# sunjay/portrayer

Measured on AMD Instinct MI355X. Metric: Mray/s (primary+shadow+secondary) at 1920x1080 SAMPLES=64, higher is better.
Workload: dtype f64; 1 GPU; big-scene (1000 analytic primitives, 3 point lights, reference scene script) 1920x1080 SAMPLES=64; width=1920, height=1080, samples=64, traversal=flat, sampling=counter-based jitter, seed 0, partition=single GPU, rays_per_frame=367740795

## Files before the change

include/portrayer_hip.h:

```cpp
#ifndef PORTRAYER_HIP_H
#define PORTRAYER_HIP_H

#include <stdint.h>

#ifdef __cplusplus
extern "C" {
#endif

#define PT_ABI_VERSION 8

enum { PT_PRIM_SPHERE = 0, PT_PRIM_TRIANGLE = 1, PT_PRIM_MESH = 2, PT_PRIM_KDMESH = 3, PT_PRIM_PLANE = 4, PT_PRIM_CUBE = 5, PT_PRIM_CYLINDER = 6, PT_PRIM_CONE = 7 };
enum { PT_TRAVERSE_FLAT = 1, PT_TRAVERSE_KD = 2, PT_TRAVERSE_HIER = 3 };
enum { PT_SAMPLE_CENTRE = 0, PT_SAMPLE_RNG = 1 };

enum {
    PT_OK = 0,
    PT_ERR_ARGUMENT = -1,
    PT_ERR_DEVICE = -2,
    PT_ERR_NO_SCENE = -3,
    PT_ERR_SLICE = -4,
    PT_ERR_SCENE = -5,
    PT_ERR_TRAVERSAL = -6
};

// ... 363 lines not shown
int pt_copy_from_device(pt_context *ctx, void *dst, const void *src, uint64_t bytes);
int pt_synchronize(pt_context *ctx);
int pt_measure_copy_bandwidth(pt_context *ctx, uint64_t bytes, int iters, double *gbps);

int pt_test_cast_rays(pt_context *ctx, uint64_t n, const double *origins, const double *directions, int any_hit,
                      double *out_t, int32_t *out_node, int32_t *out_sub);
uint64_t pt_test_scene_bytes(const pt_context *ctx);
int pt_test_scene_info(const pt_context *ctx, uint64_t out[4]);
int pt_test_vertex_box_shape(const pt_context *ctx, uint64_t out[2]);
int pt_test_math(pt_context *ctx, int op, uint64_t n, const double *a, const double *b, double *out);
int pt_test_pow_host(uint64_t n, const double *x, const double *y, double *port, double *libm);
int pt_test_libm_host(int op, uint64_t n, const double *a, const double *b, double *out);
int pt_test_work_items(const pt_render_params *params, uint32_t *sample_count, uint64_t *sample_index_sum, uint32_t *chunk_length_sum,
                       uint64_t *n_items, uint32_t *lane_pixels_chunks_samples);
typedef struct pt_scene_traits {
    int32_t traverse;
    uint32_t n_nodes, n_lights;
    int32_t has_meshes;
    int32_t has_kdmesh;
    int32_t reflective;
    int32_t reflective_opaque;
    int32_t glossy;
    int32_t area_light;
    int32_t pad;
    uint64_t instanced_tris;
} pt_scene_traits;
int pt_test_kernel_choice(const pt_scene_traits *traits, int mode, int textured, uint32_t *kernel_mode, uint32_t *kernel_variant);
int pt_test_raypk(uint64_t n, int body, const double *origins, const double *directions, const double *t_max, const float *box_lo, const float *box_hi,
                  int32_t *verdict, float *t_near, float *t_far);
int pt_test_certain_shadow(uint64_t n, int type, const double *fwd, const double *inv, const double *P, const double *L, int32_t *out_certain, int32_t *out_exact_hit);
int pt_test_pixel_beam(uint64_t n, const double *cameras, const uint32_t *pixels, const double *jitters, const float *box_lo, const float *box_hi,
                       int32_t *accept, float *bound, int32_t *walk, double *rays);
int pt_test_pixel_list_summary(pt_context *ctx, uint64_t *out);
int pt_test_film_fold_host(uint32_t n, const double *samples, const uint32_t *cuts, uint32_t n_cuts, double out_sum[3]);
int pt_test_film_moments_host(uint32_t n, const double *samples, const uint32_t *cuts, uint32_t n_cuts, double out_sum[3], double *out_q, double *out_err);
int pt_test_film_plan_host(uint32_t width, uint32_t height, const pt_rect *slice, const uint32_t *budget, uint32_t max_samples, uint32_t round, uint32_t *list, uint32_t cap,
                           uint32_t *n_out);
int pt_test_film_plan(pt_context *ctx, uint32_t width, uint32_t height, const pt_rect *slice, const uint32_t *budget, uint32_t max_samples, uint32_t round, uint32_t *list, uint32_t cap,
                      uint32_t *n_out);
int pt_test_denoise_host(uint32_t width, uint32_t height, const pt_denoise_params *params, const double *linear, const double *variance, const uint32_t *counts,
                         const pt_denoise_guides *guides, double *out_linear, double *out_variance);
int pt_test_denoise_albedo_host(uint32_t width, uint32_t height, const pt_denoise_params *params, const double *linear, const double *variance, const uint32_t *counts,
                                const pt_denoise_guides *guides, const double *albedo, double *out_linear, double *out_variance);

#ifdef __cplusplus
}
#endif
#endif
```

portrayer_amd/_hip.py:

```python
from __future__ import annotations

import ctypes as C
import os
from typing import Optional

import numpy as np

PKG_DIR = os.path.dirname(os.path.abspath(__file__))
LIB_PATH = os.path.join(PKG_DIR, "libportrayer_hip.so")

TRAVERSE_FLAT, TRAVERSE_KD, TRAVERSE_HIER = 1, 2, 3
SAMPLE_CENTRE, SAMPLE_RNG = 0, 1
OK, ERR_ARGUMENT, ERR_DEVICE, ERR_NO_SCENE, ERR_SLICE, ERR_SCENE, ERR_TRAVERSAL = 0, -1, -2, -3, -4, -5, -6
KERNEL_WAVES_MASK, KERNEL_INTERPRETER, KERNEL_PARK, KERNEL_COUNTING, KERNEL_TEXTURED, KERNEL_FORK, KERNEL_CHAIN = 15, 16, 32, 64, 128, 256, 512

_dp = C.POINTER(C.c_double)
_ip = C.POINTER(C.c_int32)
_up = C.POINTER(C.c_uint32)
_u64p = C.POINTER(C.c_uint64)
_u8p = C.POINTER(C.c_uint8)


class PortrayerHipError(RuntimeError):
    pass
# ... 162 lines not shown
DENOISE_SAME_NODE = 1
DENOISE_ALBEDO_EPS = 0.0078125


class PtDenoiseParams(C.Structure):
    _fields_ = [("iterations", C.c_int32), ("flags", C.c_uint32), ("sigma_color", C.c_double), ("sigma_plane", C.c_double), ("normal_power_log2", C.c_int32)]


class PtDenoiseGuides(C.Structure):
    _fields_ = [("position", C.c_void_p), ("normal", C.c_void_p), ("node", C.c_void_p)]


class PtStats(C.Structure):
    _fields_ = [(n, C.c_uint64) for n in ("primary", "shadow", "reflect", "refract", "depth11_skipped", "hits", "n_inner", "n_leaf",
                                          "n_analytic", "n_tri", "n_bbox", "kd_plane_miss", "stack_overflow")] + \
               [("kernel_ms", C.c_double), ("total_ms", C.c_double), ("diag", C.c_uint64 * 8), ("kernel_mode", C.c_uint32), ("kernel_variant", C.c_uint32)]

    def as_dict(self):
        d = {n: (float if n.endswith("_ms") else int)(getattr(self, n)) for n, _ in self._fields_ if n != "diag"}
        d["diag"] = [int(x) for x in self.diag]
        return d


_lib: Optional[C.CDLL] = None

EXPORTS = ["pt_abi_version", "pt_device_count", "pt_context_create", "pt_context_destroy", "pt_last_error", "pt_scene_upload",
           "pt_render", "pt_render_device", "pt_render_finish", "pt_context_stream", "pt_context_next_slot", "pt_compact_bytes", "pt_untile_device", "pt_tile_slot_pixel", "pt_untile_host", "pt_device_alloc",
           "pt_device_free", "pt_copy_to_device", "pt_copy_from_device", "pt_synchronize", "pt_measure_copy_bandwidth", "pt_test_cast_rays",
           "pt_test_math", "pt_test_work_items", "pt_node_create", "pt_node_destroy", "pt_node_last_error", "pt_node_ranks", "pt_node_uses_rccl", "pt_node_context",
           "pt_node_scene_upload", "pt_node_render", "pt_node_upload_background", "pt_node_render_resident", "pt_node_download_image",
           "pt_node_device", "pt_node_frame_begin", "pt_node_frame_end", "pt_node_frames_in_flight", "pt_node_last_frame_host_ms", "pt_node_last_frame_rank_kernel_ms", "pt_test_pow_host", "pt_test_libm_host",
           "pt_aov", "pt_aov_device", "pt_aov_finish", "pt_rays", "pt_rays_device", "pt_rays_finish", "pt_segments", "pt_segments_device",
           "pt_radiance", "pt_radiance_device", "pt_radiance_finish", "pt_scene_update", "pt_node_scene_update", "pt_scene_deform", "pt_node_scene_deform", "pt_scene_mesh_rebuildable", "pt_test_scene_bytes", "pt_test_scene_info",
           "pt_vertex_bounds_device", "pt_scene_deform_device", "pt_test_vertex_box_shape", "pt_test_raypk", "pt_test_certain_shadow", "pt_test_pixel_beam", "pt_test_pixel_list_summary",
           "pt_film_create", "pt_film_destroy", "pt_film_reset", "pt_film_add", "pt_film_add_device", "pt_film_resolve", "pt_film_resolve_device", "pt_film_counts",
           "pt_test_film_fold_host",
           "pt_film_create_moments", "pt_film_add_map", "pt_film_add_map_device", "pt_film_error", "pt_film_error_device", "pt_film_budget_device",
           "pt_test_film_moments_host", "pt_test_film_plan_host", "pt_test_film_plan",
           "pt_film_denoise", "pt_film_denoise_device", "pt_test_denoise_host",
           "pt_guides", "pt_guides_device", "pt_guides_finish", "pt_film_denoise_albedo", "pt_film_denoise_albedo_device", "pt_test_denoise_albedo_host",
           "pt_ao", "pt_ao_device", "pt_ao_finish", "pt_test_ao_rays_host", "pt_test_ao_tables",
           "pt_gather", "pt_gather_device", "pt_gather_finish", "pt_test_kernel_choice",
           "pt_chart_triangles", "pt_chart", "pt_chart_device", "pt_test_chart_host",
           "pt_direct", "pt_direct_device", "pt_direct_finish", "pt_test_direct_host"]


def header_functions():
    import re
    with open(os.path.join(os.path.dirname(os.path.dirname(os.path.abspath(__file__))), "include", "portrayer_hip.h")) as fh:
        text = re.sub(r"/\*.*?\*/", "", fh.read(), flags=re.S)
    return sorted(set(re.findall(r"\b(pt_[a-z0-9_]+)\s*\(", text)))


def missing_symbols():
    l = lib()
    return [n for n in header_functions() if not hasattr(l, n)]


def lib() -> C.CDLL:
    global _lib
    if _lib is None:
        if not os.path.exists(LIB_PATH):
            raise PortrayerHipError(f"{LIB_PATH} is missing: build it with `make` (or __graft_entry__.build()); there is no CPU fallback")
        l = C.CDLL(LIB_PATH)
        l.pt_abi_version.restype = C.c_int
        l.pt_device_count.restype = C.c_int
        l.pt_context_create.restype = C.c_int
# ... 36 lines not shown
        l.pt_context_next_slot.argtypes = [C.c_void_p]
        l.pt_compact_bytes.restype = C.c_uint64
        l.pt_compact_bytes.argtypes = [C.POINTER(PtRenderParams)]
        l.pt_untile_device.restype = C.c_int
        l.pt_untile_device.argtypes = [C.c_void_p, C.POINTER(PtRenderParams), C.c_void_p, C.c_void_p, C.c_void_p]
        l.pt_tile_slot_pixel.restype = C.c_int
        l.pt_tile_slot_pixel.argtypes = [C.POINTER(PtRenderParams), C.c_uint32, C.c_uint32, _up, _up]
        l.pt_untile_host.restype = C.c_int
        l.pt_untile_host.argtypes = [C.POINTER(PtRenderParams), _u8p, _u8p]
        l.pt_device_alloc.restype = C.c_int
        l.pt_device_alloc.argtypes = [C.c_void_p, C.c_uint64, C.POINTER(C.c_void_p)]
        l.pt_device_free.restype = C.c_int
        l.pt_device_free.argtypes = [C.c_void_p, C.c_void_p]
        l.pt_copy_to_device.restype = C.c_int
        l.pt_copy_to_device.argtypes = [C.c_void_p, C.c_void_p, C.c_void_p, C.c_uint64]
        l.pt_copy_from_device.restype = C.c_int
        l.pt_copy_from_device.argtypes = [C.c_void_p, C.c_void_p, C.c_void_p, C.c_uint64]
        l.pt_synchronize.restype = C.c_int
        l.pt_synchronize.argtypes = [C.c_void_p]
        l.pt_measure_copy_bandwidth.restype = C.c_int
        l.pt_measure_copy_bandwidth.argtypes = [C.c_void_p, C.c_uint64, C.c_int, _dp]
        l.pt_test_cast_rays.restype = C.c_int
        l.pt_test_cast_rays.argtypes = [C.c_void_p, C.c_uint64, _dp, _dp, C.c_int, _dp, _ip, _ip]
        l.pt_test_work_items.restype = C.c_int
        l.pt_test_work_items.argtypes = [C.c_void_p, C.POINTER(C.c_uint32), C.POINTER(C.c_uint64), C.POINTER(C.c_uint32), C.POINTER(C.c_uint64), C.POINTER(C.c_uint32)]
        l.pt_test_certain_shadow.restype = C.c_int
        l.pt_test_certain_shadow.argtypes = [C.c_uint64, C.c_int, _dp, _dp, _dp, _dp, _ip, _ip]
        l.pt_test_raypk.restype = C.c_int
        l.pt_test_raypk.argtypes = [C.c_uint64, C.c_int, _dp, _dp, _dp, C.POINTER(C.c_float), C.POINTER(C.c_float), _ip, C.POINTER(C.c_float), C.POINTER(C.c_float)]
        l.pt_test_pixel_list_summary.restype = C.c_int
        l.pt_test_pixel_list_summary.argtypes = [C.c_void_p, C.POINTER(C.c_uint64)]
        l.pt_test_pixel_beam.restype = C.c_int
        l.pt_test_pixel_beam.argtypes = [C.c_uint64, _dp, C.POINTER(C.c_uint32), _dp, C.POINTER(C.c_float), C.POINTER(C.c_float), _ip, C.POINTER(C.c_float), _ip, _dp]
        l.pt_test_math.restype = C.c_int
        l.pt_test_math.argtypes = [C.c_void_p, C.c_int, C.c_uint64, _dp, _dp, _dp]
        l.pt_node_create.restype = C.c_int
        l.pt_node_create.argtypes = [C.c_int, _ip, C.POINTER(C.c_void_p)]
        l.pt_node_destroy.restype = None
        l.pt_node_destroy.argtypes = [C.c_void_p]
        l.pt_node_last_error.restype = C.c_char_p
        l.pt_node_last_error.argtypes = [C.c_void_p]
        l.pt_node_ranks.restype = C.c_int
        l.pt_node_ranks.argtypes = [C.c_void_p]
        l.pt_node_uses_rccl.restype = C.c_int
        l.pt_node_uses_rccl.argtypes = [C.c_void_p]
        l.pt_node_context.restype = C.c_void_p
        l.pt_node_context.argtypes = [C.c_void_p, C.c_int]
        l.pt_node_scene_upload.restype = C.c_int
        l.pt_node_scene_upload.argtypes = [C.c_void_p, C.POINTER(PtScene), C.c_int, C.POINTER(PtKdTree)]
        l.pt_node_render.restype = C.c_int
        l.pt_node_render.argtypes = [C.c_void_p, C.POINTER(PtCamera), _dp, C.POINTER(PtRenderParams), _u8p, C.POINTER(PtStats)]
        l.pt_node_upload_background.restype = C.c_int
        l.pt_node_upload_background.argtypes = [C.c_void_p, _dp, C.POINTER(PtRenderParams), _u8p]
        l.pt_node_render_resident.restype = C.c_int
        l.pt_node_render_resident.argtypes = [C.c_void_p, C.POINTER(PtCamera), C.POINTER(PtRenderParams), C.POINTER(PtStats)]
        l.pt_node_download_image.restype = C.c_int
        l.pt_node_download_image.argtypes = [C.c_void_p, C.POINTER(PtRenderParams), _u8p]
        l.pt_node_device.restype = C.c_int
        l.pt_node_device.argtypes = [C.c_void_p, C.c_int]
        l.pt_node_frame_begin.restype = C.c_int
        l.pt_node_frame_begin.argtypes = [C.c_void_p, C.POINTER(PtCamera), C.POINTER(PtRenderParams)]
        l.pt_node_frame_end.restype = C.c_int
        l.pt_node_frame_end.argtypes = [C.c_void_p, C.POINTER(PtStats)]
        l.pt_node_frames_in_flight.restype = C.c_int
        l.pt_node_frames_in_flight.argtypes = [C.c_void_p]
        l.pt_node_last_frame_host_ms.restype = C.c_int
# ... 195 lines not shown
```

portrayer_amd/csrc/pt_api.hip:

```cpp
#include <type_traits>

#include "pt_context.h"
#include "pt_aov_inst.h"
#include "pt_guides_inst.h"
#include "pt_chart.h"
#include "pt_rays_inst.h"
#include "pt_segments_inst.h"
#include "pt_ao_inst.h"
#include "pt_direct_inst.h"
#include "pt_radiance_inst.h"
#include "pt_gather_inst.h"
#include "pt_film_inst.h"
#include "pt_film_map_inst.h"
#include "pt_denoise.h"
#include "pt_render_inst.h"
#include "pt_shade.h"
#include "pt_pixel_list.h"

template <int MODE>
__global__ void __launch_bounds__(PT_BLOCK) pt_cast_kernel(PtSceneView sc, uint64_t n, const double* o, const double* d, int any,
                                                          double* out_t, int32_t* out_node, int32_t* out_sub, unsigned int* overflow) {
    extern __shared__ uint32_t pt_lds[];
    PtStack stk;
    stk.base = pt_lds + threadIdx.x;
// ... 78 lines not shown
    PtRenderArgs r = a;
    r.tile_rank = i / slots_per_rank;
    uint32_t w = i % slots_per_rank, x, y;
    if (!pt_slot_to_pixel(r, w, &x, &y)) return;
    const uint8_t* s = gathered + 3 * (size_t)i;
    uint8_t* d = rgb + 3 * ((size_t)y * a.width + x);
    d[0] = s[0]; d[1] = s[1]; d[2] = s[2];
}

__global__ void __launch_bounds__(256) pt_occ_seed_kernel(uint32_t* __restrict__ occ, uint32_t n, int hashed, uint64_t seed, uint32_t all, uint32_t n_nodes) {
    const uint32_t i = blockIdx.x * blockDim.x + threadIdx.x;
    if (i >= n) return;
    occ[i] = hashed ? (uint32_t)(pt_rng_key(seed, i) % ((uint64_t)n_nodes + 1u)) : all + 1u;
}

__global__ void __launch_bounds__(256) pt_eye_table_kernel(const double* __restrict__ inv, double* __restrict__ tab, uint32_t n_nodes, double ex, double ey, double ez) {
    const uint32_t i = blockIdx.x * blockDim.x + threadIdx.x;
    if (i >= n_nodes) return;
    const double* m = inv + 12 * (size_t)i;
    double* o = tab + 12 * (size_t)i;
    const PtVec3 e = pt_xform_point(m, pt_v3(ex, ey, ez));
    o[0] = m[0]; o[1] = m[1]; o[2] = m[2]; o[3] = e.x;
    o[4] = m[4]; o[5] = m[5]; o[6] = m[6]; o[7] = e.y;
    o[8] = m[8]; o[9] = m[9]; o[10] = m[10]; o[11] = e.z;
}

__global__ void __launch_bounds__(256) pt_certain_table_kernel(const uint32_t* __restrict__ info, const double* __restrict__ fwd, const double* __restrict__ inv, float* __restrict__ tab,
                                                               uint32_t n_nodes) {
    const uint32_t i = blockIdx.x * blockDim.x + threadIdx.x;
    if (i >= n_nodes) return;
    pt_certain_ball(info[4 * (size_t)i], fwd + 12 * (size_t)i, inv + 12 * (size_t)i, tab + 4 * (size_t)i);
}

#define PT_PL_BLOCK 256
#define PT_PL_STACK 64
__global__ void __launch_bounds__(PT_PL_BLOCK) pt_pixel_list_kernel(PtRenderArgs a, uint32_t* __restrict__ table, uint32_t cap) {
    __shared__ uint32_t s_list[PT_PL_BLOCK / 64][PT_PL_K][64];
    __shared__ uint32_t s_stack[PT_PL_BLOCK / 64][PT_PL_STACK];
    const uint32_t wave = threadIdx.x >> 6, lane = threadIdx.x & 63u;
    const uint32_t tile_local = blockIdx.x * (PT_PL_BLOCK / 64) + wave;
    if (tile_local >= a.n_slots / 64u) return;
    const PtSceneView& sc = a.scene;
    const uint32_t slot = tile_local * 64u + lane;
    uint32_t x, y;
    pt_slot_to_pixel(a, slot, &x, &y);
    const PtBeam beam = pt_beam_setup(a.cam, (double)x, (double)y);
    uint32_t* const list = &s_list[wave][0][lane];
    uint32_t* const stack = s_stack[wave];
    uint32_t count = 0, tail = PT_PL_INF_BITS;
    if (cap > PT_PL_K) cap = PT_PL_K;
    bool overflowed = false;
    int sp = 0;
    auto add_leaf = [&](uint32_t ref, bool reached, float bound) {
        const uint32_t first = (ref & ~PT_REF_LEAF) >> 3, n = (ref & 7u) + 1u;
        for (uint32_t i = 0; i < n; i++) {
            const uint32_t node = sc.tlas_direct ? first : sc.bvh_items[first + i];
            if (reached) pt_pl_insert(list, 64u, cap, &count, &tail, pt_pl_entry(bound, node));
        }
    };
    const uint32_t root = sc.tlas_root;
    if (sc.n_nodes != 0 && root != PT_REF_EMPTY) {
        if (root & PT_REF_LEAF) add_leaf(root, true, 0.0f);
        else { stack[0] = root; sp = 1; }
    }
    while (sp > 0) {
        __builtin_amdgcn_fence(__ATOMIC_RELEASE, "wavefront");
        __builtin_amdgcn_wave_barrier();
        __builtin_amdgcn_fence(__ATOMIC_ACQUIRE, "wavefront");
        const uint32_t cur = (uint32_t)__builtin_amdgcn_readfirstlane((int)stack[sp - 1]);
        sp--;
        const pt_u32x16 nd = pt_sload_node(sc.bvh, cur);
#pragma unroll
        for (int ch = 0; ch < 2; ch++) {
            const uint32_t ref = nd[12 + ch];
            if (ref == PT_REF_EMPTY) continue;
            float lo[3], hi[3], bound = 0.0f;
#pragma unroll
            for (int k = 0; k < 3; k++) { lo[k] = pt_f32_of(nd[2 * k + ch]); hi[k] = pt_f32_of(nd[6 + 2 * k + ch]); }
            const bool reached = pt_beam_box(beam, lo, hi, &bound);
            if (!__any(reached)) continue;
            if (ref & PT_REF_LEAF) add_leaf(ref, reached, bound);
            else if (sp < PT_PL_STACK) { if (lane == 0) stack[sp] = ref; sp++; }
            else overflowed = true;
        }
    }
    uint32_t* rec = table + (size_t)slot * PT_PL_WORDS;
    uint32_t wds[PT_PL_WORDS];
    wds[0] = overflowed ? PT_PL_WALK : count;
    wds[1] = tail;
#pragma unroll
    for (uint32_t k = 0; k < PT_PL_K; k++) wds[2 + k] = k < count ? list[k * 64u] : 0u;
#pragma unroll
    for (uint32_t k = 0; k < PT_PL_WORDS; k += 4) reinterpret_cast<uint4*>(rec)[k / 4] = make_uint4(wds[k], wds[k + 1], wds[k + 2], wds[k + 3]);
}

#define PT_PASS_MISC_BYTES (256 + PT_FINE_QUEUES * PT_QUEUE_STRIDE * 4)
static size_t pt_stack_column(const PtSceneView& sc, int stack_lds_cap);

static int pt_pass_prepare(pt_context* c, PtPass& v) {
    if (v.ev0) return PT_OK;
    PT_HIP(c, hipEventCreate(&v.ev0));
    PT_HIP(c, hipEventCreate(&v.ev1));
    PT_HIP(c, hipEventCreateWithFlags(&v.copy_done, hipEventDisableTiming));
    PT_HIP(c, hipHostMalloc((void**)&v.host, 256, hipHostMallocDefault));
    return PT_OK;
}

static int pt_pass_open(pt_context* c, PtPass& v, PtRenderArgs& r, uint32_t grid, bool frames, hipStream_t stream) {
    r.n_lanes = grid * PT_BLOCK;
    int rc;
    if ((rc = pt_reserve(c, v.stack_spill, (size_t)r.n_lanes * pt_stack_column(r.scene, r.stack_lds_cap) * 4))) return rc;
    if (frames && (rc = pt_reserve(c, v.spill, pt_needs_spill(c->traits) ? (size_t)r.n_lanes * PT_SPILL_DEPTHS * PT_SPILL_STRIDE * sizeof(double) : 16))) return rc;
    if ((rc = pt_reserve(c, v.misc, PT_PASS_MISC_BYTES))) return rc;
    r.stack_spill = (uint32_t*)v.stack_spill.p;
    if (frames) r.spill = (double*)v.spill.p;
    r.overflow_flag = (unsigned int*)v.misc.p + 1;
    r.work_queues = (unsigned int*)((char*)v.misc.p + 256);
    r.fine_queues = 16;
    v.stream = stream; v.queued = true; v.closed = false;
    PT_HIP(c, hipMemsetAsync(v.misc.p, 0, PT_PASS_MISC_BYTES, stream));
    PT_HIP(c, hipEventRecord(v.ev0, stream));
    return PT_OK;
}

static int pt_pass_seal(pt_context* c, PtPass& v) {
    PT_HIP(c, hipEventRecord(v.ev1, v.stream));
    PT_HIP(c, hipMemcpyAsync(v.host, v.misc.p, 8, hipMemcpyDeviceToHost, v.stream));
// ... 259 lines not shown
            }
        }
        if (m0) v |= 2;
        if (o0) v |= 4;
        if ((m0 != 0) != (m1 != 0) || (o0 != 0) != (o1 != 0)) v |= 8;
        verdict[i] = v;
    }
    return PT_OK;
}

extern "C" int pt_test_pixel_list_summary(pt_context* c, uint64_t* out) {
    if (!c || !out) return PT_ERR_ARGUMENT;
    for (uint32_t k = 0; k < 5u + PT_PL_K; k++) out[k] = 0;
    if (c->pl_slot < 0 || c->pl_slots == 0) return PT_OK;
    PT_HIP(c, hipSetDevice(c->device));
    PT_HIP(c, hipDeviceSynchronize());
    std::vector<uint32_t> rec((size_t)c->pl_slots * PT_PL_WORDS);
    const pt_context::Slot& sl = c->slot[c->pl_slot];
    if (sl.eye_tab.bytes < c->pl_off + rec.size() * 4) return pt_fail(c, PT_ERR_ARGUMENT, "the slot's buffer no longer holds that launch's lists");
    PT_HIP(c, hipMemcpy(rec.data(), (const char*)sl.eye_tab.p + c->pl_off, rec.size() * 4, hipMemcpyDeviceToHost));
    out[0] = c->pl_slots;
    for (uint32_t i = 0; i < c->pl_slots; i++) {
        const uint32_t head = rec[(size_t)i * PT_PL_WORDS], tail = rec[(size_t)i * PT_PL_WORDS + 1];
        if (head & PT_PL_WALK) { out[3]++; continue; }
        const uint32_t n = head & 255u;
        if (n > PT_PL_K) return pt_fail(c, PT_ERR_TRAVERSAL, "a pixel list longer than its record");
        if (n == 0 && tail == PT_PL_INF_BITS) out[1]++;
        if (tail != PT_PL_INF_BITS) out[2]++;
        out[4 + n]++;
    }
    return PT_OK;
}

extern "C" int pt_test_pixel_beam(uint64_t n, const double* cameras, const uint32_t* pixels, const double* jitters, const float* box_lo, const float* box_hi,
                                  int32_t* accept, float* bound, int32_t* walk, double* rays) {
    if (!cameras || !pixels || !jitters || !box_lo || !box_hi || !accept || !bound || !walk) return PT_ERR_ARGUMENT;
    for (uint64_t i = 0; i < n; i++) {
        PtCamera cam;
        const double* cp = cameras + 19 * i;
        for (int k = 0; k < 3; k++) cam.eye[k] = cp[k];
        for (int k = 0; k < 12; k++) cam.view_to_world[k] = cp[3 + k];
        cam.fov_factor = cp[15]; cam.aspect = cp[16]; cam.width = cp[17]; cam.height = cp[18];
        const uint32_t x = pixels[2 * i], y = pixels[2 * i + 1];
        const float* lo = box_lo + 3 * i;
        const float* hi = box_hi + 3 * i;
        const PtBeam beam = pt_beam_setup(cam, (double)x, (double)y);
        float b = 0.0f;
        accept[i] = pt_beam_box(beam, lo, hi, &b) ? 1 : 0;
        bound[i] = accept[i] ? b : 0.0f;
        const PtRay r = pt_camera_ray(cam, (double)x + jitters[2 * i], (double)y + jitters[2 * i + 1]);
        if (rays) { rays[6 * i] = r.o.x; rays[6 * i + 1] = r.o.y; rays[6 * i + 2] = r.o.z; rays[6 * i + 3] = r.d.x; rays[6 * i + 4] = r.d.y; rays[6 * i + 5] = r.d.z; }
        PtRayPk q;
        int s[3];
        s[0] = pt_raypk_axis(r.o.x, r.d.x, &q.a[0], &q.b[0]); s[1] = pt_raypk_axis(r.o.y, r.d.y, &q.a[1], &q.b[1]); s[2] = pt_raypk_axis(r.o.z, r.d.z, &q.a[2], &q.b[2]);
        pt_u32x16 rec;
        for (int k = 0; k < 16; k++) rec[k] = 0u;
        for (int k = 0; k < 3; k++) {
            uint32_t l, h;
            memcpy(&l, lo + k, 4); memcpy(&h, hi + k, 4);
            rec[2 * k] = rec[2 * k + 1] = l; rec[6 + 2 * k] = rec[6 + 2 * k + 1] = h;
        }
        unsigned long long m0 = 0, m1 = 0, first = 0, o0 = 0, o1 = 0;
        pt_slab_pk2<PT_OCT_MIXED>(rec, q, INFINITY, &m0, &m1, &first);
        o0 = m0; o1 = m1;
        if (s[0] && s[1] && s[2]) {
            switch ((s[0] == 2 ? 1 : 0) | (s[1] == 2 ? 2 : 0) | (s[2] == 2 ? 4 : 0)) {
                case 0: pt_slab_pk2<0>(rec, q, INFINITY, &o0, &o1, &first); break;
                case 1: pt_slab_pk2<1>(rec, q, INFINITY, &o0, &o1, &first); break;
                case 2: pt_slab_pk2<2>(rec, q, INFINITY, &o0, &o1, &first); break;
                case 3: pt_slab_pk2<3>(rec, q, INFINITY, &o0, &o1, &first); break;
                case 4: pt_slab_pk2<4>(rec, q, INFINITY, &o0, &o1, &first); break;
                case 5: pt_slab_pk2<5>(rec, q, INFINITY, &o0, &o1, &first); break;
                case 6: pt_slab_pk2<6>(rec, q, INFINITY, &o0, &o1, &first); break;
                default: pt_slab_pk2<7>(rec, q, INFINITY, &o0, &o1, &first); break;
            }
        }
        walk[i] = (m0 ? 1 : 0) | (o0 ? 2 : 0);
    }
    return PT_OK;
}

extern "C" int pt_test_certain_shadow(uint64_t n, int type, const double* fwd, const double* inv, const double* P, const double* L, int32_t* out_certain, int32_t* out_exact_hit) {
    if (!fwd || !inv || !P || !L || !out_certain || !out_exact_hit || type < 0 || type > 7) return PT_ERR_ARGUMENT;
    for (uint64_t i = 0; i < n; i++) {
        float ball[4];
        pt_certain_ball((uint32_t)type, fwd + 12 * i, inv + 12 * i, ball);
        const PtVec3 p = pt_v3(P[3 * i], P[3 * i + 1], P[3 * i + 2]), l = pt_v3(L[3 * i], L[3 * i + 1], L[3 * i + 2]);
        out_certain[i] = ball[3] > 0.0f && pt_certain_lane(ball, (float)p.x, (float)p.y, (float)p.z, (float)l.x, (float)l.y, (float)l.z) ? 1 : 0;
        PtRay r;
        r.o = p;
        const PtVec3 hit_to_light = l - p;
        r.d = hit_to_light / pt_length(hit_to_light);
        const PtRay local = pt_ray_to_local(inv + 12 * i, r);
        double t;
        uint32_t part = 0;
        out_exact_hit[i] = pt_unit_prim_hit((uint32_t)type, local, PT_EPSILON, INFINITY, &t, &part) ? 1 : 0;
    }
    return PT_OK;
}

static bool pt_kd_semantics(int mode) { return mode == PT_MODE_KD || mode == PT_MODE_KD_NOMESH || mode == PT_MODE_KD_MESH; }
static int pt_stack_lds_cap(const PtSceneView& sc, size_t block_budget, size_t frame_bytes) {
    int lds_cap = block_budget > frame_bytes ? (int)((block_budget - frame_bytes) / (PT_BLOCK * 4)) : 0;
    lds_cap = std::max(lds_cap, 2);
    if (const char* e = getenv("PORTRAYER_LDS_STACK")) lds_cap = std::max(1, atoi(e));
    int cap = std::min(lds_cap, sc.stack_cap);
    if (pt_kd_semantics(sc.mode)) cap = std::max(cap, (sc.stack_cap + 63) / 64 + 2);
    return cap;
}
static size_t pt_stack_column(const PtSceneView& sc, int stack_lds_cap) {
    const int wave_rows = std::min(std::max(8, (sc.stack_cap + 63) / 64), std::max(stack_lds_cap, 8));
// ... 152 lines not shown
        }
        occ_seed = true;
    }
    if ((rc = pt_reserve(c, sl.misc, misc_head + occ_bytes))) return rc;
    if ((rc = pt_reserve(c, sl.accum, (size_t)a.n_slots * a.n_chunks * 3 * sizeof(double)))) return rc;
    a.accum = (double*)sl.accum.p;
#ifndef PT_NO_EYE_TABLE
    const bool eye_table = a.scene.mode == PT_MODE_FLAT_NOMESH && a.scene.n_nodes > 0;
#else
    const bool eye_table = false;
#endif
#ifndef PT_NO_CERTAIN_SHADOW
    const bool certain_table = a.scene.mode == PT_MODE_FLAT_NOMESH && a.scene.n_nodes > 0 && occ_bytes != 0;
#else
    const bool certain_table = false;
#endif
#ifndef PT_NO_PIXEL_LISTS
    const bool list_header = eye_table;
#ifdef PT_PIXEL_LIST_STATS
    const bool list_reader = true;
#else
    const bool list_reader = !stats;
#endif
    bool pixel_lists = eye_table && list_reader && (a.run_variant == PT_RUN_LINE3 || a.run_variant == PT_RUN_LINE4 || a.run_variant == PT_RUN_LINE5) && a.k_log2 + a.c_log2 == 6u &&
                       a.scene.n_nodes <= PT_PL_MAX_NODES && a.n_slots != 0;
    if (const char* e = getenv("PORTRAYER_PIXEL_LISTS")) if (atoi(e) <= 0) pixel_lists = false;
    uint32_t list_cap = PT_PL_K;
    if (const char* e = getenv("PORTRAYER_PIXEL_LIST_CAP"); e && *e) {
        char* end = nullptr;
        const unsigned long long k = strtoull(e, &end, 10);
        if (end == e || *end || k > PT_PL_K) return pt_fail(c, PT_ERR_ARGUMENT, std::string("PORTRAYER_PIXEL_LIST_CAP=") + e + ": expected 0 .. " + std::to_string(PT_PL_K));
        list_cap = (uint32_t)k;
    }
#else
    const bool list_header = false, pixel_lists = false;
    const uint32_t list_cap = 0;
#endif
    const size_t list_off = pt_pl_header_offset((uint32_t)a.scene.n_nodes);
    a.eye_tab = nullptr;
    if (eye_table || certain_table) {
        if ((rc = pt_reserve(c, sl.eye_tab, list_header ? list_off + pt_pl_bytes(pixel_lists ? a.n_slots : 0u) : (size_t)a.scene.n_nodes * (12 * sizeof(double) + 4 * sizeof(float))))) return rc;
        a.eye_tab = (const double*)sl.eye_tab.p;
    }
    a.spill = (double*)sl.spill.p;
    a.stack_spill = (uint32_t*)sl.stack_spill.p;
    a.work_counter = (unsigned int*)sl.misc.p;
    a.overflow_flag = (unsigned int*)sl.misc.p + 1;
    a.counters = (PtCounters*)((char*)sl.misc.p + 256);
    a.work_queues = (unsigned int*)((char*)sl.misc.p + 256 + sizeof(PtCounters));
    a.occluders = occ_bytes ? (uint32_t*)((char*)sl.misc.p + misc_head) : nullptr;
    a.occ_row = std::max<uint32_t>(a.div_tiles_x.d / std::max<uint32_t>(a.tile_ranks, 1u), 1u);
    c->last_mode = (uint32_t)a.scene.mode;
    c->last_variant = pt_choice_variant(choice, tex) | (stats ? PT_KERNEL_COUNTING : 0u);
    PT_HIP(c, hipMemsetAsync(sl.misc.p, 0, misc_head + occ_bytes, stream));
    if (occ_seed) {
        const uint32_t n_occ = (uint32_t)(occ_bytes / 4);
        hipLaunchKernelGGL(pt_occ_seed_kernel, dim3((n_occ + 255) / 256), dim3(256), 0, stream, a.occluders, n_occ, occ_hashed ? 1 : 0, occ_seed_value, occ_all, a.scene.n_nodes);
        PT_HIP(c, hipGetLastError());
        if (getenv("PORTRAYER_VERBOSE")) fprintf(stderr, "[pt_render] occluder table: %u entries seeded (PORTRAYER_OCC_SEED=%s)\n", n_occ, getenv("PORTRAYER_OCC_SEED"));
    }
    sl.mode = c->last_mode; sl.variant = c->last_variant; sl.counted = stats;
    PT_HIP(c, hipEventRecord(sl.ev0, stream));
    if (a.n_items) {
        if (eye_table) {
            hipLaunchKernelGGL(pt_eye_table_kernel, dim3((a.scene.n_nodes + 255) / 256), dim3(256), 0, stream, a.scene.inv, (double*)sl.eye_tab.p, (uint32_t)a.scene.n_nodes,
                               a.cam.eye[0], a.cam.eye[1], a.cam.eye[2]);
            PT_HIP(c, hipGetLastError());
        }
        if (certain_table) {
            hipLaunchKernelGGL(pt_certain_table_kernel, dim3((a.scene.n_nodes + 255) / 256), dim3(256), 0, stream, a.scene.info, a.scene.fwd, a.scene.inv, (float*)((double*)sl.eye_tab.p + 12 * (size_t)a.scene.n_nodes),
                               (uint32_t)a.scene.n_nodes);
            PT_HIP(c, hipGetLastError());
        }
        if (list_header) {
            uint32_t* const header = (uint32_t*)((char*)sl.eye_tab.p + list_off);
            PT_HIP(c, hipMemsetD32Async((hipDeviceptr_t)header, pixel_lists ? 1 : 0, 16, stream));
            if (pixel_lists) {
                const uint32_t tiles = a.n_slots / 64u;
                hipLaunchKernelGGL(pt_pixel_list_kernel, dim3((tiles + PT_PL_BLOCK / 64 - 1) / (PT_PL_BLOCK / 64)), dim3(PT_PL_BLOCK), 0, stream, a, header + 16, list_cap);
                PT_HIP(c, hipGetLastError());
            }
        }
        c->pl_slot = pixel_lists ? slot_index : -1; c->pl_slots = a.n_slots; c->pl_off = list_off + 64;
        PT_HIP(c, pt_dispatch(a, stats, c->n_cu, stream, &grid, true));
        hipLaunchKernelGGL(pt_finish_kernel, dim3((a.n_slots + PT_BLOCK - 1) / PT_BLOCK), dim3(PT_BLOCK), 0, stream, a);
        PT_HIP(c, hipGetLastError());
    }
    PT_HIP(c, hipEventRecord(sl.ev1, stream));
    PT_HIP(c, hipMemcpyAsync(sl.host, sl.misc.p, stats ? PT_SLOT_BYTES : 8, hipMemcpyDeviceToHost, stream));
    PT_HIP(c, hipEventRecord(sl.copy_done, stream));
    return PT_OK;
}

static int pt_collect_stats(pt_context* c, pt_stats* st, int slot_index) {
    pt_context::Slot& sl = c->slot[slot_index];
    if (st) memset(st, 0, sizeof *st);
    unsigned int head[2];
    memcpy(head, sl.host, sizeof head);
    if (st) {
        float ms = 0.f;
        PT_HIP(c, hipEventElapsedTime(&ms, sl.ev0, sl.ev1));
        st->kernel_ms = ms;
        if (sl.counted) {
            PtCounters h;
            memcpy(&h, sl.host + 256, sizeof h);
            st->primary = h.primary; st->shadow = h.shadow; st->reflect = h.reflect; st->refract = h.refract;
            st->depth11_skipped = h.depth11_skipped; st->hits = h.hits; st->n_inner = h.n_inner; st->n_leaf = h.n_leaf;
            st->n_analytic = h.n_analytic; st->n_tri = h.n_tri; st->n_bbox = h.n_bbox; st->kd_plane_miss = h.kd_plane_miss;
            st->stack_overflow = h.stack_overflow;
            for (int k = 0; k < 8; k++) st->diag[k] = h.diag[k];
        }
        if (head[1] && !st->stack_overflow) st->stack_overflow = 1;
        st->kernel_mode = sl.mode; st->kernel_variant = sl.variant;
    }
    if (head[1] & 2u) return pt_fail(c, PT_ERR_TRAVERSAL, "fork / join of refracted subtrees stalled (a lane waited for a colour nobody was computing): results invalid");
    if (head[1] & 4u) return pt_fail(c, PT_ERR_TRAVERSAL, "a tree walk did not end (watchdog): results invalid");
// ... 1581 lines not shown
```

portrayer_amd/csrc/pt_context.h:

```cpp
#pragma once
#include <hip/hip_runtime.h>

#include <algorithm>
#include <chrono>
#include <cmath>
#include <cstdio>
#include <cstring>
#include <string>
#include <vector>

#include "../../include/portrayer_hip.h"
#include "pt_build.h"
#include "pt_bvh.h"
#include "pt_shade.h"

struct PtBuf {
    void* p = nullptr;
    size_t bytes = 0;
    PtBuf() = default;
    PtBuf(const PtBuf&) = delete;
    PtBuf& operator=(const PtBuf&) = delete;
    ~PtBuf() { if (p) hipFree(p); }
};

// ... 27 lines not shown
struct pt_film;
struct pt_context {
    int device = 0;
    int n_cu = 0;
    std::string err;
    PtBuf inv, fwd, nrm, info, tri_v, tri_e, tri_leaf, tri_n, meshes, materials, lights, bvh, bvh4, bvh_items, kd, kd_items;
    PtBuf mat_maps, uv_trans, tex, tex_rgb, srgb_lut, tri_uv, texview, mkd, mkd_items;
    PtBuf node_box, kd_box, mkd_box, mkd_item_box, kd_ref;
    PtBuf g_inv, g_fwd, g_nrm, chain_off, chain, dfs_rank, hier_rec, own_inv;
    PtBuf bg, rgb, linear, misc;
    PtSceneTraits traits = {};
    uint32_t launch_seq = 0;
    PtSceneView view;
    bool have_scene = false;
    struct Slot {
        PtBuf spill, stack_spill, accum, misc;
        PtBuf eye_tab;
        hipStream_t stream = nullptr;
        hipEvent_t ev0 = nullptr, ev1 = nullptr;
        hipEvent_t copy_done = nullptr;
        unsigned char* host = nullptr;
        bool pending = false, counted = false;
        uint32_t mode = 0, variant = 0;
        std::chrono::steady_clock::time_point t_start;
    };
    static constexpr int PT_SLOTS = 2;
    Slot slot[PT_SLOTS];
    int slot_next = 0;
    int slot_oldest = 0;
    uint32_t last_mode = 0, last_variant = 0;
    int pl_slot = -1;
    uint32_t pl_slots = 0;
    size_t pl_off = 0;
    struct Aov {
        PtPass pass;
        PtBuf out[6];
        PtBuf albedo;
        bool guides = false;
        PtBuf chart_owner, chart_uv, chart_covered;
        bool chart = false;
    } aov;
    struct Rays {
        PtPass pass;
        PtBuf in[2], in_t_max, out[7];
        PtRaySort sort;
    } rays;
    struct Radiance {
        PtPass pass;
        PtBuf in[3], out;
        PtRaySort sort;
    } radiance;
    PtPass* const passes[3] = {&aov.pass, &rays.pass, &radiance.pass};
    std::vector<pt_film*> films;
    pt_film* film_open = nullptr;
    struct Resident {
        int traverse = 0;
        uint32_t n_nodes = 0, n_graph = 0, n_lights = 0;
        std::vector<uint32_t> info;
        std::vector<PtBuildBox> mesh_box;
        std::vector<PtBuildBox> tri_box;
        size_t mesh_tris = 0;
        std::vector<uint32_t> chain_off, chain;
        size_t tlas_first = 0, tlas_cap = 0;
        size_t tlas_items = 0;
        size_t tree_nodes = 0;
        int tlas_leaf = 1, collapse_mode = 1;
// ... 62 lines not shown
```

portrayer_amd/csrc/pt_pixel_list.h:

```cpp
#pragma once

#include "pt_scene_view.h"

#ifndef PT_PL_K
#define PT_PL_K 6u
#endif
#define PT_PL_WORDS (PT_PL_K <= 6u ? 8u : 16u)
static_assert(PT_PL_K >= 1u && PT_PL_K <= 14u, "a record is 8 or 16 words: head, tail bound, entries");
#define PT_PL_WALK 0x80000000u
#define PT_PL_MAX_NODES 65536u
#define PT_PL_INF_BITS 0x7F800000u

PT_HD size_t pt_pl_header_offset(uint32_t n_nodes) { return ((size_t)n_nodes * (12 * sizeof(double) + 4 * sizeof(float)) + 63u) & ~(size_t)63u; }
PT_HD size_t pt_pl_bytes(uint32_t n_slots) { return 64u + (size_t)n_slots * (PT_PL_WORDS * 4u); }

struct PtBeamAxis {
    int neg;
    float a1, a2;
    float be1, be2;
    float bf1, bf2;
};
struct PtBeam {
    PtBeamAxis ax[3];
    float lmin;
};

PT_HD float pt_f32_below(double v) {
    float f = (float)v;
    if ((double)f > v) {
        const uint32_t u = __builtin_bit_cast(uint32_t, f);
        f = f > 0.0f ? __builtin_bit_cast(float, u - 1u) : (f < 0.0f ? __builtin_bit_cast(float, u + 1u) : -1.401298464324817e-45f);
    }
    return f;
}
PT_HD float pt_f32_above(double v) { return -pt_f32_below(-v); }

PT_HD double pt_beam_view_x(const PtCamera& c, double x) {
    double ndc_x = x / c.width;
    return (2.0 * ndc_x - 1.0) * c.aspect * c.fov_factor;
}
PT_HD double pt_beam_view_y(const PtCamera& c, double y) {
    double ndc_y = y / c.height;
    return (1.0 - 2.0 * ndc_y) * c.fov_factor;
}
PT_HD void pt_beam_corner(const PtCamera& c, double view_x, double view_y, double D[3]) {
    PtVec3 eye = pt_v3(c.eye[0], c.eye[1], c.eye[2]);
    PtVec3 world = pt_xform_point(c.view_to_world, pt_v3(view_x, view_y, -1.0));
    PtVec3 d = world - eye;
    D[0] = d.x; D[1] = d.y; D[2] = d.z;
}

PT_HD PtBeam pt_beam_setup(const PtCamera& c, double px, double py) {
    double lo[3], hi[3];
    bool finite = true;
    const double vx[2] = {pt_beam_view_x(c, px), pt_beam_view_x(c, px + 1.0)}, vy[2] = {pt_beam_view_y(c, py), pt_beam_view_y(c, py + 1.0)};
    for (int k = 0; k < 4; k++) {
        double D[3];
        pt_beam_corner(c, vx[k & 1], vy[k >> 1], D);
        for (int a = 0; a < 3; a++) {
            finite = finite && fabs(D[a]) < INFINITY;
            if (k == 0) { lo[a] = hi[a] = D[a]; }
            else { lo[a] = fmin(lo[a], D[a]); hi[a] = fmax(hi[a], D[a]); }
        }
    }
    double lmax2 = 0.0, lmin2 = 0.0;
    for (int a = 0; a < 3; a++) {
        const double m = fmax(fabs(lo[a]), fabs(hi[a]));
        lmax2 += m * m;
        const double n = (lo[a] > 0.0) ? lo[a] : ((hi[a] < 0.0) ? -hi[a] : 0.0);
        lmin2 += n * n;
    }
    const double lmax = sqrt(lmax2) * (1.0 + 1e-12), lmin = sqrt(lmin2) * (1.0 - 1e-12);
    const double zt = 4e-18 * lmax;
    const double c0 = lmin > 0.0 ? 5e-20 / lmin : (double)INFINITY;
    PtBeam b;
    for (int a = 0; a < 3; a++) {
        PtBeamAxis& x = b.ax[a];
        x.neg = 0; x.a1 = x.a2 = 0.0f; x.be1 = x.be2 = -INFINITY; x.bf1 = x.bf2 = INFINITY;
        double dl, dh, o;
        if (!finite) continue;
        if (lo[a] > zt && hi[a] >= lo[a]) { o = c.eye[a]; dl = lo[a]; dh = hi[a]; }
        else if (hi[a] < -zt && hi[a] >= lo[a]) { x.neg = 1; o = -c.eye[a]; dl = -hi[a]; dh = -lo[a]; }
        else continue;
        const float a1 = (float)((1.0 / dh) * (1.0 - 0x1p-18)), a2 = (float)((1.0 / dl) * (1.0 + 0x1p-18));
        const double m = (6e-7 * fabs(o)) * (double)a2 + c0 + 1e-12 * (fabs(o) * (double)a2);
        const float be1 = pt_f32_below(-o * (double)a1 - m), be2 = pt_f32_below(-o * (double)a2 - m);
        const float bf1 = pt_f32_above(-o * (double)a1 + m), bf2 = pt_f32_above(-o * (double)a2 + m);
        if (!(a1 > 0.0f && a2 <= 1e19f && fabsf(be1) < INFINITY && fabsf(be2) < INFINITY && fabsf(bf1) < INFINITY && fabsf(bf2) < INFINITY)) { x.neg = 0; continue; }
// ... 46 lines not shown
```

Baseline: 61140 Mray/s.

## Build per-pixel candidate lists with wave-wide breadth-first tile-beam BVH traversal

Replaces the per-wave depth-first stack walk in the pixel-list kernel with a breadth-first traversal. All 64 lanes expand pending BVH nodes together against a shared 8x8 tile beam, then leaf candidates are buffered in LDS and flushed through each pixel's own beam test. The aim is to raise lane utilisation and cut divergent serial node visits while building the lists. In exchange it uses more LDS per wave (a 1024-entry pending queue plus a candidate buffer) with 64-thread blocks, and it falls back to the walk path when the queue overflows. It also adds test hooks for rectangular beams and for reading back list records.

```diff
diff --git a/include/portrayer_hip.h b/include/portrayer_hip.h
--- a/include/portrayer_hip.h
+++ b/include/portrayer_hip.h
@@ -419,6 +419,9 @@
 int pt_test_pixel_beam(uint64_t n, const double *cameras, const uint32_t *pixels, const double *jitters, const float *box_lo, const float *box_hi,
                        int32_t *accept, float *bound, int32_t *walk, double *rays);
 int pt_test_pixel_list_summary(pt_context *ctx, uint64_t *out);
+int pt_test_rect_beam(uint64_t n, const double *cameras, const uint32_t *rects, const double *offsets, const float *box_lo, const float *box_hi,
+                      int32_t *accept, float *bound, int32_t *walk, double *rays);
+int pt_test_pixel_list_records(pt_context *ctx, uint32_t *out, uint64_t words, uint64_t *info);
 int pt_test_film_fold_host(uint32_t n, const double *samples, const uint32_t *cuts, uint32_t n_cuts, double out_sum[3]);
 int pt_test_film_moments_host(uint32_t n, const double *samples, const uint32_t *cuts, uint32_t n_cuts, double out_sum[3], double *out_q, double *out_err);
 int pt_test_film_plan_host(uint32_t width, uint32_t height, const pt_rect *slice, const uint32_t *budget, uint32_t max_samples, uint32_t round, uint32_t *list, uint32_t cap,
diff --git a/portrayer_amd/_hip.py b/portrayer_amd/_hip.py
--- a/portrayer_amd/_hip.py
+++ b/portrayer_amd/_hip.py
@@ -218,7 +218,7 @@
            "pt_node_device", "pt_node_frame_begin", "pt_node_frame_end", "pt_node_frames_in_flight", "pt_node_last_frame_host_ms", "pt_node_last_frame_rank_kernel_ms", "pt_test_pow_host", "pt_test_libm_host",
            "pt_aov", "pt_aov_device", "pt_aov_finish", "pt_rays", "pt_rays_device", "pt_rays_finish", "pt_segments", "pt_segments_device",
            "pt_radiance", "pt_radiance_device", "pt_radiance_finish", "pt_scene_update", "pt_node_scene_update", "pt_scene_deform", "pt_node_scene_deform", "pt_scene_mesh_rebuildable", "pt_test_scene_bytes", "pt_test_scene_info",
-           "pt_vertex_bounds_device", "pt_scene_deform_device", "pt_test_vertex_box_shape", "pt_test_raypk", "pt_test_certain_shadow", "pt_test_pixel_beam", "pt_test_pixel_list_summary",
+           "pt_vertex_bounds_device", "pt_scene_deform_device", "pt_test_vertex_box_shape", "pt_test_raypk", "pt_test_certain_shadow", "pt_test_pixel_beam", "pt_test_pixel_list_summary", "pt_test_rect_beam", "pt_test_pixel_list_records",
            "pt_film_create", "pt_film_destroy", "pt_film_reset", "pt_film_add", "pt_film_add_device", "pt_film_resolve", "pt_film_resolve_device", "pt_film_counts",
            "pt_test_film_fold_host",
            "pt_film_create_moments", "pt_film_add_map", "pt_film_add_map_device", "pt_film_error", "pt_film_error_device", "pt_film_budget_device",
@@ -321,6 +321,10 @@
         l.pt_test_pixel_list_summary.argtypes = [C.c_void_p, C.POINTER(C.c_uint64)]
         l.pt_test_pixel_beam.restype = C.c_int
         l.pt_test_pixel_beam.argtypes = [C.c_uint64, _dp, C.POINTER(C.c_uint32), _dp, C.POINTER(C.c_float), C.POINTER(C.c_float), _ip, C.POINTER(C.c_float), _ip, _dp]
+        l.pt_test_rect_beam.restype = C.c_int
+        l.pt_test_rect_beam.argtypes = l.pt_test_pixel_beam.argtypes
+        l.pt_test_pixel_list_records.restype = C.c_int
+        l.pt_test_pixel_list_records.argtypes = [C.c_void_p, C.POINTER(C.c_uint32), C.c_uint64, C.POINTER(C.c_uint64)]
         l.pt_test_math.restype = C.c_int
         l.pt_test_math.argtypes = [C.c_void_p, C.c_int, C.c_uint64, _dp, _dp, _dp]
         l.pt_node_create.restype = C.c_int
diff --git a/portrayer_amd/csrc/pt_api.hip b/portrayer_amd/csrc/pt_api.hip
--- a/portrayer_amd/csrc/pt_api.hip
+++ b/portrayer_amd/csrc/pt_api.hip
@@ -134,9 +134,129 @@
     pt_certain_ball(info[4 * (size_t)i], fwd + 12 * (size_t)i, inv + 12 * (size_t)i, tab + 4 * (size_t)i);
 }
 
+#ifndef PT_PL_DEPTH_FIRST
+#define PT_PL_BLOCK 64
+#define PT_PL_PENDING 1024u
+#define PT_PL_STEP_CANDS 128u
+#define PT_PL_CANDS 128u
+#define PT_PL_WAVE_SYNC() do { __builtin_amdgcn_fence(__ATOMIC_RELEASE, "wavefront"); __builtin_amdgcn_wave_barrier(); __builtin_amdgcn_fence(__ATOMIC_ACQUIRE, "wavefront"); } while (0)
+static __device__ __forceinline__ float pt_pl_scalar(float v) { return __builtin_bit_cast(float, __builtin_amdgcn_readfirstlane(__builtin_bit_cast(int, v))); }
+static __device__ __forceinline__ uint32_t pt_pl_lanes_below(unsigned long long m) { return __builtin_amdgcn_mbcnt_hi((uint32_t)(m >> 32), __builtin_amdgcn_mbcnt_lo((uint32_t)m, 0u)); }
+__global__ void __launch_bounds__(PT_PL_BLOCK) pt_pixel_list_kernel(PtRenderArgs a, uint32_t* __restrict__ table, uint32_t cap, uint32_t pend_cap) {
+    __shared__ uint32_t s_list[PT_PL_BLOCK / 64][PT_PL_K][64];
+    __shared__ uint32_t s_pend[PT_PL_BLOCK / 64][PT_PL_PENDING];
+    __shared__ uint4 s_cand[PT_PL_BLOCK / 64][PT_PL_CANDS * 2u];
+    static_assert(PT_PL_CANDS >= PT_PL_STEP_CANDS, "the empty buffer takes a step's candidates");
+    const uint32_t wave = threadIdx.x >> 6, lane = threadIdx.x & 63u;
+    const uint32_t tile_local = PT_UNIFORM_U32(blockIdx.x * (PT_PL_BLOCK / 64) + wave);
+    if (tile_local >= a.n_slots / 64u) return;
+    const PtSceneView& sc = a.scene;
+    const uint32_t slot = tile_local * 64u + lane;
+    uint32_t x, y, tx, ty;
+    pt_slot_to_pixel(a, slot, &x, &y);
+    pt_slot_to_pixel(a, tile_local * 64u, &tx, &ty);
+    const PtBeam beam = pt_beam_setup(a.cam, (double)x, (double)y);
+    PtBeam tile = pt_beam_setup(a.cam, (double)tx, (double)ty, 8.0, 8.0);
+#pragma unroll
+    for (int k = 0; k < 3; k++) {
+        PtBeamAxis& t = tile.ax[k];
+        t.neg = __builtin_amdgcn_readfirstlane(t.neg);
+        t.a1 = pt_pl_scalar(t.a1); t.a2 = pt_pl_scalar(t.a2); t.be1 = pt_pl_scalar(t.be1); t.be2 = pt_pl_scalar(t.be2); t.bf1 = pt_pl_scalar(t.bf1); t.bf2 = pt_pl_scalar(t.bf2);
+    }
+    tile.lmin = pt_pl_scalar(tile.lmin);
+    uint32_t* const list = &s_list[wave][0][lane];
+    uint32_t* const pend = s_pend[wave];
+    uint4* const cand = s_cand[wave];
+    uint32_t count = 0, tail = PT_PL_INF_BITS;
+    if (cap > PT_PL_K) cap = PT_PL_K;
+    if (pend_cap > PT_PL_PENDING) pend_cap = PT_PL_PENDING;
+    bool overflowed = false;
+    uint32_t n_pend = 0, n_cand = 0;
+    const bool direct = sc.tlas_direct != 0;
+    const uint32_t root = sc.tlas_root;
+    if (sc.n_nodes != 0 && root != PT_REF_EMPTY) {
+        if (root & PT_REF_LEAF) {
+            const uint32_t first = (root & ~PT_REF_LEAF) >> 3, n = direct ? 1u : (root & 7u) + 1u;
+            for (uint32_t i = 0; i < n; i++) pt_pl_insert(list, 64u, cap, &count, &tail, pt_pl_entry(0.0f, direct ? first : sc.bvh_items[first + i]));
+        } else {
+            if (lane == 0) pend[0] = root;
+            n_pend = 1;
+        }
+    }
+    auto flush = [&]() {
+        PT_PL_WAVE_SYNC();
+        for (uint32_t j = 0; j < n_cand; j++) {
+            const uint4 c0 = cand[2u * j], c1 = cand[2u * j + 1u];
+            const float lo[3] = {pt_f32_of(c0.y), pt_f32_of(c0.z), pt_f32_of(c0.w)}, hi[3] = {pt_f32_of(c1.x), pt_f32_of(c1.y), pt_f32_of(c1.z)};
+            float bound = 0.0f;
+            if (pt_beam_box(beam, lo, hi, &bound)) pt_pl_insert(list, 64u, cap, &count, &tail, pt_pl_entry(bound, c0.x));
+        }
+        n_cand = 0;
+    };
+    const uint32_t width = direct ? 64u : PT_PL_STEP_CANDS / 16u;
+    while (n_pend > 0) {
+        if (n_cand > PT_PL_CANDS - PT_PL_STEP_CANDS) flush();
+        PT_PL_WAVE_SYNC();
+        const uint32_t take = n_pend < width ? n_pend : width;
+        n_pend -= take;
+        uint32_t ref[2] = {PT_REF_EMPTY, PT_REF_EMPTY};
+        uint32_t nd[12] = {};
+        bool reached[2] = {false, false};
+        if (lane < take) {
+            const uint4* const p = reinterpret_cast<const uint4*>(sc.bvh) + 4u * (size_t)pend[n_pend + lane];
+            const uint4 q0 = p[0], q1 = p[1], q2 = p[2];
+            const uint2 q3 = *reinterpret_cast<const uint2*>(p + 3);
+            nd[0] = q0.x; nd[1] = q0.y; nd[2] = q0.z; nd[3] = q0.w; nd[4] = q1.x; nd[5] = q1.y; nd[6] = q1.z; nd[7] = q1.w; nd[8] = q2.x; nd[9] = q2.y; nd[10] = q2.z; nd[11] = q2.w;
+            ref[0] = q3.x; ref[1] = q3.y;
+#pragma unroll
+            for (int ch = 0; ch < 2; ch++) {
+                if (ref[ch] == PT_REF_EMPTY) continue;
+                float lo[3], hi[3], bound;
+#pragma unroll
+                for (int k = 0; k < 3; k++) { lo[k] = pt_f32_of(nd[2 * k + ch]); hi[k] = pt_f32_of(nd[6 + 2 * k + ch]); }
+                reached[ch] = pt_beam_box(tile, lo, hi, &bound);
+            }
+        }
+        const bool inner0 = reached[0] && !(ref[0] & PT_REF_LEAF), inner1 = reached[1] && !(ref[1] & PT_REF_LEAF);
+        const unsigned long long m0 = __ballot(inner0), m1 = __ballot(inner1);
+        const uint32_t n0 = (uint32_t)__builtin_popcountll(m0), n1 = (uint32_t)__builtin_popcountll(m1);
+        if (n_pend + n0 + n1 > pend_cap) { overflowed = true; break; }
+        if (inner0) pend[n_pend + pt_pl_lanes_below(m0)] = ref[0];
+        if (inner1) pend[n_pend + n0 + pt_pl_lanes_below(m1)] = ref[1];
+        n_pend += n0 + n1;
+#pragma unroll
+        for (int ch = 0; ch < 2; ch++) {
+            const bool leaf = reached[ch] && (ref[ch] & PT_REF_LEAF);
+            const uint32_t first = (ref[ch] & ~PT_REF_LEAF) >> 3, n = !leaf ? 0u : (direct ? 1u : (ref[ch] & 7u) + 1u);
+            for (uint32_t i = 0; i < 8u; i++) {
+                const bool mine = i < n;
+                const unsigned long long m = __ballot(mine);
+                if (m == 0) break;
+                if (mine) {
+                    const uint32_t at = 2u * (n_cand + pt_pl_lanes_below(m));
+                    cand[at] = make_uint4(direct ? first : sc.bvh_items[first + i], nd[ch], nd[2 + ch], nd[4 + ch]);
+                    cand[at + 1u] = make_uint4(nd[6 + ch], nd[8 + ch], nd[10 + ch], 0u);
+                }
+                n_cand += (uint32_t)__builtin_popcountll(m);
+            }
+        }
+    }
+    if (!overflowed && n_cand) flush();
+    uint32_t* rec = table + (size_t)slot * PT_PL_WORDS;
+    uint32_t wds[PT_PL_WORDS];
+    wds[0] = overflowed ? PT_PL_WALK : count;
+    wds[1] = tail;
+#pragma unroll
+    for (uint32_t k = 0; k < PT_PL_K; k++) wds[2 + k] = k < count ? list[k * 64u] : 0u;
+#pragma unroll
+    for (uint32_t k = 2 + PT_PL_K; k < PT_PL_WORDS; k++) wds[k] = 0u;
+#pragma unroll
+    for (uint32_t k = 0; k < PT_PL_WORDS; k += 4) reinterpret_cast<uint4*>(rec)[k / 4] = make_uint4(wds[k], wds[k + 1], wds[k + 2], wds[k + 3]);
+}
+#else
 #define PT_PL_BLOCK 256
 #define PT_PL_STACK 64
-__global__ void __launch_bounds__(PT_PL_BLOCK) pt_pixel_list_kernel(PtRenderArgs a, uint32_t* __restrict__ table, uint32_t cap) {
+__global__ void __launch_bounds__(PT_PL_BLOCK) pt_pixel_list_kernel(PtRenderArgs a, uint32_t* __restrict__ table, uint32_t cap, uint32_t pend_cap) {
     __shared__ uint32_t s_list[PT_PL_BLOCK / 64][PT_PL_K][64];
     __shared__ uint32_t s_stack[PT_PL_BLOCK / 64][PT_PL_STACK];
     const uint32_t wave = threadIdx.x >> 6, lane = threadIdx.x & 63u;
@@ -195,6 +315,7 @@
 #pragma unroll
     for (uint32_t k = 0; k < PT_PL_WORDS; k += 4) reinterpret_cast<uint4*>(rec)[k / 4] = make_uint4(wds[k], wds[k + 1], wds[k + 2], wds[k + 3]);
 }
+#endif
 
 #define PT_PASS_MISC_BYTES (256 + PT_FINE_QUEUES * PT_QUEUE_STRIDE * 4)
 static size_t pt_stack_column(const PtSceneView& sc, int stack_lds_cap);
@@ -520,19 +641,19 @@
     return PT_OK;
 }
 
-extern "C" int pt_test_pixel_beam(uint64_t n, const double* cameras, const uint32_t* pixels, const double* jitters, const float* box_lo, const float* box_hi,
-                                  int32_t* accept, float* bound, int32_t* walk, double* rays) {
-    if (!cameras || !pixels || !jitters || !box_lo || !box_hi || !accept || !bound || !walk) return PT_ERR_ARGUMENT;
+static int pt_test_beam_cases(uint64_t n, const double* cameras, const uint32_t* rects, uint32_t stride, const double* jitters, const float* box_lo, const float* box_hi,
+                              int32_t* accept, float* bound, int32_t* walk, double* rays) {
+    if (!cameras || !rects || !jitters || !box_lo || !box_hi || !accept || !bound || !walk) return PT_ERR_ARGUMENT;
     for (uint64_t i = 0; i < n; i++) {
         PtCamera cam;
         const double* cp = cameras + 19 * i;
         for (int k = 0; k < 3; k++) cam.eye[k] = cp[k];
         for (int k = 0; k < 12; k++) cam.view_to_world[k] = cp[3 + k];
         cam.fov_factor = cp[15]; cam.aspect = cp[16]; cam.width = cp[17]; cam.height = cp[18];
-        const uint32_t x = pixels[2 * i], y = pixels[2 * i + 1];
+        const uint32_t x = rects[stride * i], y = rects[stride * i + 1];
         const float* lo = box_lo + 3 * i;
         const float* hi = box_hi + 3 * i;
-        const PtBeam beam = pt_beam_setup(cam, (double)x, (double)y);
+        const PtBeam beam = stride == 4u ? pt_beam_setup(cam, (double)x, (double)y, (double)rects[4 * i + 2], (double)rects[4 * i + 3]) : pt_beam_setup(cam, (double)x, (double)y);
         float b = 0.0f;
         accept[i] = pt_beam_box(beam, lo, hi, &b) ? 1 : 0;
         bound[i] = accept[i] ? b : 0.0f;
@@ -565,6 +686,29 @@
         }
         walk[i] = (m0 ? 1 : 0) | (o0 ? 2 : 0);
     }
+    return PT_OK;
+}
+extern "C" int pt_test_pixel_beam(uint64_t n, const double* cameras, const uint32_t* pixels, const double* jitters, const float* box_lo, const float* box_hi,
+                                  int32_t* accept, float* bound, int32_t* walk, double* rays) {
+    return pt_test_beam_cases(n, cameras, pixels, 2u, jitters, box_lo, box_hi, accept, bound, walk, rays);
+}
+extern "C" int pt_test_rect_beam(uint64_t n, const double* cameras, const uint32_t* rects, const double* offsets, const float* box_lo, const float* box_hi,
+                                 int32_t* accept, float* bound, int32_t* walk, double* rays) {
+    return pt_test_beam_cases(n, cameras, rects, 4u, offsets, box_lo, box_hi, accept, bound, walk, rays);
+}
+
+extern "C" int pt_test_pixel_list_records(pt_context* c, uint32_t* out, uint64_t words, uint64_t* info) {
+    if (!c || !info) return PT_ERR_ARGUMENT;
+    info[0] = 0; info[1] = PT_PL_WORDS; info[2] = PT_PL_K; info[3] = c->pl_nodes;
+    if (c->pl_slot < 0 || c->pl_slots == 0) return PT_OK;
+    info[0] = c->pl_slots;
+    const size_t need = (size_t)c->pl_slots * PT_PL_WORDS;
+    if (!out || words < need) return PT_OK;
+    PT_HIP(c, hipSetDevice(c->device));
+    PT_HIP(c, hipDeviceSynchronize());
+    const pt_context::Slot& sl = c->slot[c->pl_slot];
+    if (sl.eye_tab.bytes < c->pl_off + need * 4) return pt_fail(c, PT_ERR_ARGUMENT, "the slot's buffer no longer holds that launch's lists");
+    PT_HIP(c, hipMemcpy(out, (const char*)sl.eye_tab.p + c->pl_off, need * 4, hipMemcpyDeviceToHost));
     return PT_OK;
 }
 
@@ -783,9 +927,16 @@
         if (end == e || *end || k > PT_PL_K) return pt_fail(c, PT_ERR_ARGUMENT, std::string("PORTRAYER_PIXEL_LIST_CAP=") + e + ": expected 0 .. " + std::to_string(PT_PL_K));
         list_cap = (uint32_t)k;
     }
+    uint32_t list_pending = 1024u;
+    if (const char* e = getenv("PORTRAYER_PIXEL_LIST_PENDING"); e && *e) {
+        char* end = nullptr;
+        const unsigned long long k = strtoull(e, &end, 10);
+        if (end == e || *end || k < 1u || k > list_pending) return pt_fail(c, PT_ERR_ARGUMENT, std::string("PORTRAYER_PIXEL_LIST_PENDING=") + e + ": expected 1 .. " + std::to_string(list_pending));
+        list_pending = (uint32_t)k;
+    }
 #else
     const bool list_header = false, pixel_lists = false;
-    const uint32_t list_cap = 0;
+    const uint32_t list_cap = 0, list_pending = 0;
 #endif
     const size_t list_off = pt_pl_header_offset((uint32_t)a.scene.n_nodes);
     a.eye_tab = nullptr;
@@ -828,11 +979,11 @@
             PT_HIP(c, hipMemsetD32Async((hipDeviceptr_t)header, pixel_lists ? 1 : 0, 16, stream));
             if (pixel_lists) {
                 const uint32_t tiles = a.n_slots / 64u;
-                hipLaunchKernelGGL(pt_pixel_list_kernel, dim3((tiles + PT_PL_BLOCK / 64 - 1) / (PT_PL_BLOCK / 64)), dim3(PT_PL_BLOCK), 0, stream, a, header + 16, list_cap);
+                hipLaunchKernelGGL(pt_pixel_list_kernel, dim3((tiles + PT_PL_BLOCK / 64 - 1) / (PT_PL_BLOCK / 64)), dim3(PT_PL_BLOCK), 0, stream, a, header + 16, list_cap, list_pending);
                 PT_HIP(c, hipGetLastError());
             }
         }
-        c->pl_slot = pixel_lists ? slot_index : -1; c->pl_slots = a.n_slots; c->pl_off = list_off + 64;
+        c->pl_slot = pixel_lists ? slot_index : -1; c->pl_slots = a.n_slots; c->pl_off = list_off + 64; c->pl_nodes = (uint32_t)a.scene.n_nodes;
         PT_HIP(c, pt_dispatch(a, stats, c->n_cu, stream, &grid, true));
         hipLaunchKernelGGL(pt_finish_kernel, dim3((a.n_slots + PT_BLOCK - 1) / PT_BLOCK), dim3(PT_BLOCK), 0, stream, a);
         PT_HIP(c, hipGetLastError());
diff --git a/portrayer_amd/csrc/pt_context.h b/portrayer_amd/csrc/pt_context.h
--- a/portrayer_amd/csrc/pt_context.h
+++ b/portrayer_amd/csrc/pt_context.h
@@ -83,6 +83,7 @@
     int pl_slot = -1;
     uint32_t pl_slots = 0;
     size_t pl_off = 0;
+    uint32_t pl_nodes = 0;
     struct Aov {
         PtPass pass;
         PtBuf out[6];
diff --git a/portrayer_amd/csrc/pt_pixel_list.h b/portrayer_amd/csrc/pt_pixel_list.h
--- a/portrayer_amd/csrc/pt_pixel_list.h
+++ b/portrayer_amd/csrc/pt_pixel_list.h
@@ -50,10 +50,10 @@
     D[0] = d.x; D[1] = d.y; D[2] = d.z;
 }
 
-PT_HD PtBeam pt_beam_setup(const PtCamera& c, double px, double py) {
+PT_HD PtBeam pt_beam_setup(const PtCamera& c, double px, double py, double nx = 1.0, double ny = 1.0) {
     double lo[3], hi[3];
     bool finite = true;
-    const double vx[2] = {pt_beam_view_x(c, px), pt_beam_view_x(c, px + 1.0)}, vy[2] = {pt_beam_view_y(c, py), pt_beam_view_y(c, py + 1.0)};
+    const double vx[2] = {pt_beam_view_x(c, px), pt_beam_view_x(c, px + nx)}, vy[2] = {pt_beam_view_y(c, py), pt_beam_view_y(c, py + ny)};
     for (int k = 0; k < 4; k++) {
         double D[3];
         pt_beam_corner(c, vx[k & 1], vy[k >> 1], D);
```

After: 63680 Mray/s (median of 6 runs). 4.1% higher.
